# wenxiaoshuai/Points-Matching

Measured on AMD Instinct MI355X. Metric: descriptor-pair distances/s (BF-L2 2-NN + ratio stage); RANSAC hypotheses/s in `ransac`, higher is better.
Workload: dtype f32

## Files before the change

include/pm.h:

```cpp
#ifndef PM_H_
#define PM_H_

#include <stddef.h>
#include <stdint.h>

#ifdef __cplusplus
extern "C" {
#endif

#define PM_VERSION_MAJOR 0
#define PM_VERSION_MINOR 1

typedef enum pm_status {
    PM_OK            =  0,
    PM_E_INVALID     = -1,
    PM_E_TOO_FEW     = -2,
    PM_E_NO_MODEL    = -3,
    PM_E_HIP         = -4,
    PM_E_NOMEM       = -5,
    PM_E_UNSUPPORTED = -6
} pm_status;

typedef struct pm_match {
    int32_t queryIdx;
// ... 6 lines not shown

int  pm_ctx_create(int device, pm_ctx** out);
int  pm_ctx_destroy(pm_ctx* ctx);
int  pm_ctx_set_stream(pm_ctx* ctx, void* hip_stream);
int  pm_ctx_synchronize(pm_ctx* ctx);
int  pm_device_alloc(pm_ctx* ctx, size_t bytes, void** d_out);
int  pm_device_free(pm_ctx* ctx, void* d_ptr);
int  pm_device_upload(pm_ctx* ctx, void* d_dst, const void* src, size_t bytes);
int  pm_device_download(pm_ctx* ctx, void* dst, const void* d_src, size_t bytes);
int  pm_ctx_timing_enable(pm_ctx* ctx, int enable);
int  pm_ctx_timing_reset(pm_ctx* ctx);
int  pm_ctx_timing_get(pm_ctx* ctx, const char* kernel, double* mean_ms, int* launches);
int  pm_ctx_knn_diag_enable(pm_ctx* ctx, int enable);
int  pm_ctx_knn_stats(pm_ctx* ctx, int* rescans, int* nonfinite);
int  pm_ctx_knn_route(pm_ctx* ctx, int* route);
int  pm_ctx_filter_fusion_status(pm_ctx* ctx, int* gave_up);
enum {
    PM_OPT_RANSAC_PATH    = 1,
    PM_OPT_SCORE_OPERANDS = 2,
    PM_OPT_HAMMING_ROUTE  = 3,
    PM_OPT_KNN_F16_WAVES  = 4,
    PM_OPT_KNN_STAGING    = 6,
    PM_OPT_KNN_WG_PER_CU  = 7,
    PM_OPT_FILTER_FUSION  = 5,
    PM_OPT_KNN_XCD_TILE   = 8,
    PM_OPT_KNN_GENERAL_F16 = 9,
    PM_OPT_KNN_SEEDED     = 10,
    PM_OPT_KNN_U8_GROUP   = 11,
    PM_OPT_KNN_RING       = 12,
    PM_OPT_KNN_U8_REFINE  = 13,
    PM_OPT_KNN_RING_PROLOGUE = 14,
    PM_OPT_KNN_WIDE       = 15,
    PM_OPT_KNN_PREP_ROWS  = 16,
    PM_OPT_RANSAC_FORM    = 17,
    PM_OPT_RANSAC_WG_IDS  = 18,
    PM_OPT_HAMMING_REFINE = 19,
    PM_OPT_KNN_SUPERTILE  = 20,
    PM_OPT_FEAT_CAPACITY  = 21,
    PM_OPT_COUNT_         = 22
};
int  pm_ctx_set_option(pm_ctx* ctx, int option, int value);
int  pm_ctx_get_option(pm_ctx* ctx, int option, int* value);
const char* pm_last_error(void);
const char* pm_status_string(int status);
int  pm_version(void);

#define PM_MAX_K 16
#define PM_KNN_FORCE_EXACT  1
#define PM_KNN_FORCE_F32    2
#define PM_KNN_HINT_INTEGER 4
#define PM_KNN_HINT_U8      8
#define PM_KNN_HINT_UNIT_NORM 16
int pm_bf_knn_l2_f32(pm_ctx* ctx, const float* q, int nq, const float* t, int nt,
                     int dim, int k, int flags, pm_match* out);
// ... 379 lines not shown
```

points_matching_amd/api.py:

```python
import ctypes as C
import os

import numpy as np

_HERE = os.path.dirname(os.path.abspath(__file__))
LIB_PATH = os.environ.get("PM_LIB_PATH") or os.path.join(_HERE, "libpm_hip.so")

MATCH_DTYPE = np.dtype([("queryIdx", "<i4"), ("trainIdx", "<i4"), ("imgIdx", "<i4"),
                        ("distance", "<f4")])
PM_MAX_K = 16
PM_KNN_FORCE_EXACT = 1
PM_KNN_FORCE_F32 = 2
PM_KNN_HINT_INTEGER = 4
PM_KNN_HINT_U8 = 8
PM_KNN_HINT_UNIT_NORM = 16
PM_CROSS_RATIO_FWD = 1
PM_CROSS_RATIO_REV = 2
PM_GUIDE_F_SAMPSON = 0
PM_GUIDE_F_SYM = 1
PM_GUIDE_H = 2
PM_ERR_SAMPSON = 0
PM_ERR_SYM_EPIPOLAR = 1
PM_ERR_REPROJ = 2
PM_AFFINE_FULL = 0
PM_AFFINE_PARTIAL = 1
PM_OK, PM_E_INVALID, PM_E_TOO_FEW, PM_E_NO_MODEL, PM_E_HIP, PM_E_NOMEM, PM_E_UNSUPPORTED = \
    0, -1, -2, -3, -4, -5, -6

EXPORTS = [
    "pm_ctx_create", "pm_ctx_destroy", "pm_ctx_set_stream", "pm_ctx_synchronize",
    "pm_ctx_timing_enable", "pm_ctx_timing_reset", "pm_ctx_timing_get", "pm_ctx_knn_diag_enable", "pm_ctx_knn_stats", "pm_ctx_knn_route",
    "pm_ctx_filter_fusion_status",
    "pm_last_error",
    "pm_status_string", "pm_version",
    "pm_bf_knn_l2_f32", "pm_bf_knn_l2_f32_dev", "pm_bf_knn_hamming_u8", "pm_bf_knn_hamming_u8_dev",
    "pm_filter_midpoint", "pm_filter_ratio", "pm_match_indices", "pm_gather_points",
    "pm_format_match_list",
    "pm_filter_ratio_gather_dev", "pm_filter_midpoint_gather_dev", "pm_concat_points_dev",
    "pm_ransac_fundamental", "pm_ransac_score_dev", "pm_ransac_score_devn", "pm_ransac_model_from_hyp",
    "pm_ransac_model_from_key_dev", "pm_ransac_run_dev", "pm_ransac_shard_parts_dev", "pm_ransac_finish_parts_dev",
    "pm_ctx_set_option", "pm_ctx_get_option", "pm_bf_knn_l2_ratio_dev",
    "pm_flann_build", "pm_flann_destroy", "pm_flann_knn_l2_f32", "pm_flann_knn_l2_f32_dev", "pm_flann_export",
    "pm_mgpu_create", "pm_mgpu_destroy", "pm_mgpu_size", "pm_mgpu_ctx", "pm_mgpu_ransac_fundamental", "pm_mgpu_match_ransac",
    "pm_mgpu_lane_ctx", "pm_mgpu_set_lanes", "pm_mgpu_set_train", "pm_mgpu_set_train_dev", "pm_mgpu_submit_dev", "pm_mgpu_collect",
    "pm_mgpu_allgather_latency", "pm_mgpu_batch_run", "pm_mgpu_batch_set_option",
    "pm_batch_create", "pm_batch_destroy", "pm_batch_run", "pm_batch_set_option", "pm_batch_set_desc_type", "pm_batch_set_host_threads",
# ... 84 lines not shown
PM_OPT_KNN_STAGING = 6
PM_OPT_KNN_WG_PER_CU = 7
PM_OPT_KNN_XCD_TILE = 8
PM_OPT_KNN_GENERAL_F16 = 9
PM_OPT_KNN_SEEDED = 10
PM_OPT_KNN_U8_GROUP = 11
PM_OPT_KNN_RING = 12
PM_OPT_KNN_U8_REFINE = 13
PM_OPT_KNN_RING_PROLOGUE = 14
PM_OPT_KNN_WIDE = 15
PM_OPT_KNN_PREP_ROWS = 16
PM_OPT_RANSAC_FORM = 17
PM_OPT_RANSAC_WG_IDS = 18
PM_OPT_HAMMING_REFINE = 19
PM_OPT_KNN_SUPERTILE = 20
PM_OPT_FEAT_CAPACITY = 21


_lib = None


def lib():
    global _lib
    if _lib is None:
        if not os.path.exists(LIB_PATH):
            raise PmError(PM_E_UNSUPPORTED,
                          "%s is missing: run `python -m points_matching_amd.build`" % LIB_PATH)
        try:
            import torch
        except ImportError:
# ... 213 lines not shown
                                                mask_len, C.c_void_p(dninl_ptr or 0), C.c_void_p(dntotal_ptr or 0)))

    def knn_diag_enable(self, on=True):
        _check(lib().pm_ctx_knn_diag_enable(self._h, int(on)))

    def filter_fusion_gave_up(self):
        g = C.c_int()
        _check(lib().pm_ctx_filter_fusion_status(self._h, C.byref(g)))
        return g.value

    def knn_stats(self):
        r, nf = C.c_int(), C.c_int()
        _check(lib().pm_ctx_knn_stats(self._h, C.byref(r), C.byref(nf)))
        rt = C.c_int()
        _check(lib().pm_ctx_knn_route(self._h, C.byref(rt)))
        return {"rescans": r.value, "nonfinite": nf.value, "route": rt.value}

    def filter_ratio_gather_dev(self, dknn_ptr, nq, k, ratio, dkp1_ptr, dkp2_ptr, dgood_ptr, dxy1_ptr,
                                dxy2_ptr, dn_ptr):
        _check(lib().pm_filter_ratio_gather_dev(self._h, C.c_void_p(dknn_ptr), nq, k, C.c_float(ratio),
                                                C.c_void_p(dkp1_ptr), C.c_void_p(dkp2_ptr),
                                                C.c_void_p(dgood_ptr), C.c_void_p(dxy1_ptr),
                                                C.c_void_p(dxy2_ptr), C.c_void_p(dn_ptr)))

    def filter_cross_gather_dev(self, dfwd_ptr, nq, kf, drev_ptr, nt, kr, cross_flags, ratio, dkp1_ptr, dkp2_ptr, dgood_ptr,
                                dxy1_ptr, dxy2_ptr, dn_ptr):
        _check(lib().pm_filter_cross_gather_dev(self._h, C.c_void_p(dfwd_ptr), nq, kf, C.c_void_p(drev_ptr), nt, kr,
                                                cross_flags, C.c_float(ratio), C.c_void_p(dkp1_ptr or 0),
                                                C.c_void_p(dkp2_ptr or 0), C.c_void_p(dgood_ptr), C.c_void_p(dxy1_ptr or 0),
                                                C.c_void_p(dxy2_ptr or 0), C.c_void_p(dn_ptr)))

# ... 906 lines not shown
```

points_matching_amd/csrc/knn_l2.hip:

```cpp
#include <cstdlib>

#include "knn_shared.hpp"

namespace {

using namespace pm_knn;

constexpr int TILE_T = 64;
constexpr int PM_U8_FUSED_MAX_NQ = 768;
__host__ inline bool u8_fused_by_default(int nq) { return nq <= PM_U8_FUSED_MAX_NQ; }
constexpr float KNN_INF = __builtin_inff();

__device__ __forceinline__ uint32_t f32_bits(float f) { return __float_as_uint(f); }

__device__ __forceinline__ uint64_t knn_key(float dist, int idx)
{
    uint32_t b = (dist != dist) ? 0x7FC00000u : f32_bits(dist);
    return (static_cast<uint64_t>(b) << 32) | static_cast<uint32_t>(idx);
}

template <bool VEC4>
__device__ __forceinline__ float l2sqr_canonical(const float* __restrict__ a,
                                                 const float* __restrict__ b, int dim)
{
// ... 115 lines not shown
#pragma unroll
        for (int k = 0; k < 8; ++k) {
            float x = ALIGNED ? (k < 4 ? a[k & 3] : b[k & 3]) : e[k];
            const bool in = ALIGNED ? (c + (k & ~3) < dim) : (c + k < dim);
            v[k] = (live && in) ? x : 0.f;
        }
    }
};

template <bool SEEDED, int DP, bool ALIGNED>
__global__ __launch_bounds__(256) void knn_l2_prep16(const float* __restrict__ Q, int nq, int nq_pad,
                                                     const float* __restrict__ T, int nt, int nt_pad, int dim,
                                                     float* __restrict__ qnorm, float* __restrict__ tnorm,
                                                     _Float16* __restrict__ Qh, _Float16* __restrict__ Th,
                                                     float* __restrict__ seeds,
                                                     unsigned long long* __restrict__ stats, unsigned epoch)
{
    typedef F16Rows<DP> G;
    constexpr int ROWH = SEEDED ? DP : G::ROWH;
    constexpr int NCB = G::NCB;
    __shared__ unsigned wmax[4];
    __shared__ unsigned wbad[4];
    const int sub = threadIdx.x & 15, grp = threadIdx.x >> 4;
    const int qblocks = nq_pad / 64;
    const bool is_t = static_cast<int>(blockIdx.x) >= qblocks;
    const float* x = is_t ? T : Q;
    const int n = is_t ? nt : nq;
    float* norm = is_t ? tnorm : qnorm;
    _Float16* xh = is_t ? Th : Qh;
    const int row0 = (is_t ? blockIdx.x - qblocks : blockIdx.x) * 64;
    unsigned mx = 0u, bad = 0u;
// ... 59 lines not shown
        }
    }
#pragma unroll
    for (int o = 32; o > 0; o >>= 1) {
        mx = max(mx, static_cast<unsigned>(__shfl_xor(static_cast<int>(mx), o, 64)));
        bad |= static_cast<unsigned>(__shfl_xor(static_cast<int>(bad), o, 64));
    }
    if ((threadIdx.x & 63) == 0) { wmax[threadIdx.x >> 6] = mx; wbad[threadIdx.x >> 6] = bad; }
    __syncthreads();
    if (threadIdx.x == 0) {
        mx = max(max(wmax[0], wmax[1]), max(wmax[2], wmax[3]));
        bad = wbad[0] | wbad[1] | wbad[2] | wbad[3];
        const unsigned long long tag = static_cast<unsigned long long>(epoch) << 32;
        if (is_t) atomicMax(&stats[0], tag | mx);
        if (bad) atomicMax(&stats[1], tag | static_cast<unsigned long long>(bad == 1u ? 3u : bad));
    }
}

template <int ITERS>
__global__ __launch_bounds__(256) void knn_l2_prep8(const float* __restrict__ Q, int nq, int nq_pad,
                                                    const float* __restrict__ T, int nt, int nt_pad, int dim,
                                                    float* __restrict__ qnorm, float* __restrict__ tnorm,
                                                    uint2* __restrict__ Q8, uint2* __restrict__ T8,
                                                    int* __restrict__ seeds, unsigned long long* __restrict__ stats,
                                                    unsigned epoch, int t_wide, uint2* __restrict__ Qf)
{
    __shared__ unsigned wbad[4];
    const int sub = threadIdx.x & 15, grp = threadIdx.x >> 4;
    const int qblocks = nq_pad / (16 * ITERS);
    const bool is_t = static_cast<int>(blockIdx.x) >= qblocks;
// ... 318 lines not shown
        }
    }
#pragma unroll
    for (int o = 32; o > 0; o >>= 1) bad |= static_cast<unsigned>(__shfl_xor(static_cast<int>(bad), o, 64));
    if ((threadIdx.x & 63) == 0) wbad[threadIdx.x >> 6] = bad;
    __syncthreads();
    if (threadIdx.x == 0) {
        const unsigned long long tag = static_cast<unsigned long long>(epoch) << 32;
        bad = wbad[0] | wbad[1] | wbad[2] | wbad[3];
        if (blockIdx.x == 0) {
            atomicMax(&stats[0], tag | f32_bits(BOUND2));
            atomicMax(&stats[1], tag | 2ull);
        }
        if (bad) atomicMax(&stats[1], tag | 3ull);
    }
}

template <int KM>
struct BestN {
    uint64_t k[KM];
    float d[KM];
    __device__ __forceinline__ void init()
    {
#pragma unroll
        for (int i = 0; i < KM; ++i) { k[i] = ~0ull; d[i] = KNN_INF; }
    }
    __device__ __forceinline__ void insert(uint64_t key, float dist)
    {
        if (key < k[KM - 1]) {
            k[KM - 1] = key; d[KM - 1] = dist;
// ... 843 lines not shown
    }
    if (++ctx->kf_epoch >= (1u << 24)) {
        PM_HIP_CHECK(hipMemsetAsync(ctx->kf_tile, 0, static_cast<size_t>(ctx->kf_cap) * 12, ctx->stream));
        ctx->kf_epoch = 1;
    }
    fz.tile = ctx->kf_tile;
    fz.tilecnt = reinterpret_cast<unsigned*>(ctx->kf_tile + ctx->kf_cap);
    fz.err = reinterpret_cast<unsigned*>(ctx->knn_stats) + 12;
    fz.epoch = ctx->kf_epoch;
    return PM_OK;
}

int knn_l2_enqueue(pm_ctx* ctx, const float* dq, int nq, const float* dt, int nt, int dim, int k, int flags, pm_match* dout,
                   KnnFuse* fuse, const uint8_t* uq = nullptr, const uint8_t* ut = nullptr)
{
    const bool u8in = uq != nullptr;
    if (u8in) {
        const bool al = ((reinterpret_cast<uintptr_t>(uq) | reinterpret_cast<uintptr_t>(ut)) & 3) == 0;
        if (!(k <= 4 && (dim % 4) == 0 && dim <= 128 && nt >= 1 && al)) return 2;
        flags = PM_KNN_HINT_U8;
    }

    const bool aligned16 = u8in || ((reinterpret_cast<uintptr_t>(dq) | reinterpret_cast<uintptr_t>(dt)) & 15) == 0;
    const bool vec = (dim % 4) == 0 && aligned16;
    const bool narrow = vec && dim <= 128;
    const bool wide16 = !narrow && !(flags & PM_KNN_FORCE_F32) && ctx->opts[PM_OPT_KNN_WIDE] != 1;
    const bool fast = !(flags & PM_KNN_FORCE_EXACT) && (k <= 2 || (k <= 4 && ctx->opts[PM_OPT_KNN_WIDE] != 1)) && dim <= 256 &&
                      nt >= 1 && (narrow || wide16) && (dim >= 4 || !vec);
    if (!fast) {
        if (u8in) return 2;
// ... 114 lines not shown
    void* Qf = qfb ? pm::arena_take(ctx, qfb) : nullptr;
    PM_REQUIRE(qnorm && tnorm && (!want32 || cval32) && (!want16 || (cval16 && Qh && Th)) && (!sdb || seeds) && (!qfb || Qf),
               PM_E_NOMEM, "scratch arena too small");
    KnnFuse fz{};
    if (fuse) {
        fz = *fuse;
        fz.pk = static_cast<unsigned long long*>(pm::arena_take(ctx, pkb));
        PM_REQUIRE(fz.pk != nullptr, PM_E_NOMEM, "scratch arena too small");
        rc = kf_prepare(ctx, nq, fz, (u8r && u8_int_refine) ? 16 : 32);
        if (rc != PM_OK) return rc;
    }
    g32.cand = cval32;
    g16.cand = cval16;

    unsigned long long* stats = ctx->knn_stats;
    PM_REFUSE_CAPTURE(ctx);
    if (++ctx->knn_epoch == 0u) {
        PM_HIP_CHECK(hipMemsetAsync(stats, 0, 32, ctx->stream));
        ctx->knn_epoch = 1u;
    }
    const unsigned epoch = ctx->knn_epoch;
    unsigned* diag = nullptr;
    if (ctx->knn_diag) {
        diag = ctx->knn_diag_words;
        PM_HIP_CHECK(hipMemsetAsync(diag, 0, 12, ctx->stream));
    }
    {
        pm::ScopedKernelTime t(ctx, "knn_l2_prep");
        if (u8in)
            hipLaunchKernelGGL(knn_l2_prep8_u8, dim3(nq_pad / 64 + nt_pad / 64), dim3(256), 0, ctx->stream, uq, nq, nq_pad, ut, nt,
                               nt_pad, dim, qnorm, tnorm, reinterpret_cast<uint2*>(Qh), reinterpret_cast<uint2*>(Th),
                               static_cast<int*>(seeds), t_wide, static_cast<uint2*>(Qf));
        else if (u8r && ctx->opts[PM_OPT_KNN_PREP_ROWS] != 1)
            hipLaunchKernelGGL(knn_l2_prep8<1>, dim3(nq_pad / 16 + nt_pad / 16), dim3(256), 0, ctx->stream, dq, nq, nq_pad, dt,
                               nt, nt_pad, dim, qnorm, tnorm, reinterpret_cast<uint2*>(Qh), reinterpret_cast<uint2*>(Th),
                               static_cast<int*>(seeds), stats, epoch, t_wide, static_cast<uint2*>(Qf));
        else if (u8r)
            hipLaunchKernelGGL(knn_l2_prep8<4>, dim3(nq_pad / 64 + nt_pad / 64), dim3(256), 0, ctx->stream, dq, nq, nq_pad, dt,
                               nt, nt_pad, dim, qnorm, tnorm, reinterpret_cast<uint2*>(Qh), reinterpret_cast<uint2*>(Th),
                               static_cast<int*>(seeds), stats, epoch, t_wide, static_cast<uint2*>(Qf));
        else if (f16s)
            hipLaunchKernelGGL((knn_l2_prep16<true, 128, true>), dim3(nq_pad / 64 + nt_pad / 64), dim3(256), 0, ctx->stream, dq, nq,
                               nq_pad, dt, nt, nt_pad, dim, qnorm, tnorm, Qh, Th, static_cast<float*>(seeds), stats, epoch);
        else if (unit_hint) {
#define PM_PREP16U(DP_, AL_)                                                                                              \
    hipLaunchKernelGGL((knn_l2_prep16u<DP_, AL_>), dim3(nq_pad / 64 + nt_pad / 64), dim3(256), 0, ctx->stream, dq, nq, nq_pad, dt, \
                       nt, nt_pad, dim, qnorm, tnorm, Qh, Th, stats, epoch)
            if (dp16 == 128) { if (vec) PM_PREP16U(128, true); else PM_PREP16U(128, false); }
            else { if (vec) PM_PREP16U(256, true); else PM_PREP16U(256, false); }
#undef PM_PREP16U
        }
        else if (want16) {
#define PM_PREP16(DP_, AL_)                                                                                               \
    hipLaunchKernelGGL((knn_l2_prep16<false, DP_, AL_>), dim3(nq_pad / 64 + nt_pad / 64), dim3(256), 0, ctx->stream, dq, nq,    \
                       nq_pad, dt, nt, nt_pad, dim, qnorm, tnorm, Qh, Th, nullptr, stats, epoch)
            if (dp16 == 128) { if (vec) PM_PREP16(128, true); else PM_PREP16(128, false); }
            else { if (vec) PM_PREP16(256, true); else PM_PREP16(256, false); }
#undef PM_PREP16
        }
        else
            hipLaunchKernelGGL(knn_l2_prep, dim3((nq + 63) / 64 + (nt + 63) / 64), dim3(256), 0, ctx->stream, dq, nq, dt,
                               nt, dim, qnorm, tnorm, stats, epoch);
        if (route == ROUTE_AUTO && !gen32 && !unit_hint) {
#define PM_PREP16G(DP_, AL_)                                                                                              \
    hipLaunchKernelGGL((knn_l2_prep16g<DP_, AL_>), dim3(nq_pad / 64 + nt_pad / 64), dim3(256), 0, ctx->stream, dq, nq, nq_pad, dt, \
                       nt, nt_pad, dim, qnorm, tnorm, Qh, Th, stats, epoch)
            if (dp16 == 128) { if (vec) PM_PREP16G(128, true); else PM_PREP16G(128, false); }
            else { if (vec) PM_PREP16G(256, true); else PM_PREP16G(256, false); }
#undef PM_PREP16G
        }
        else if (gen32)
            hipLaunchKernelGGL(knn_gen_off, dim3(1), dim3(64), 0, ctx->stream, stats, epoch);
        PM_HIP_CHECK(hipGetLastError());
    }
    if (u8r) {
        rc = launch_coarse_u8(ctx, Qh, Qf, Th, static_cast<const int*>(seeds), nq, nq_pad, nt, splits16, g16.tiles_per_split,
                              reinterpret_cast<int*>(cval16), g16.slots, u8_group, u8_form);
        if (rc != PM_OK) return rc;
    } else if (f16s) {
        rc = launch_coarse_f16s(ctx, Qh, Th, static_cast<const float*>(seeds), nq, nq_pad, nt, splits16, g16.tiles_per_split,
                                ~g16.lid_mask, cval16, g16.slots);
        if (rc != PM_OK) return rc;
    } else if (want16) {
        rc = launch_coarse_f16(ctx, Qh, Th, nq, nq_pad, nt, splits16, g16.tiles_per_split, ~g16.lid_mask, cval16,
                               g16.slots, stats, epoch, route == ROUTE_AUTO ? 1 : 0, dp16);
        if (rc != PM_OK) return rc;
    }
    if (want32) {
        rc = launch_coarse_f32(ctx, dq, nq, dt, nt, dim, tnorm, splits32, g32.tiles_per_split, ~g32.lid_mask, cval32,
// ... 29 lines not shown
#define PM_REFINE4(VEC_, NS_, FUSE_, GEN_) do { if (k <= 2) PM_REFINE5(VEC_, NS_, FUSE_, GEN_, 2); else PM_REFINE5(VEC_, NS_, false, GEN_, 4); } while (0)
#define PM_REFINE3(NS_, FUSE_, GEN_) do { if (vec) PM_REFINE4(true, NS_, FUSE_, GEN_); else PM_REFINE4(false, NS_, FUSE_, GEN_); } while (0)
#define PM_REFINE2(NS_, FUSE_) do { if (route == ROUTE_AUTO) PM_REFINE3(NS_, FUSE_, true); else PM_REFINE3(NS_, FUSE_, false); } while (0)
#define PM_REFINE(NS_) do { if (fuse) PM_REFINE2(NS_, true); else PM_REFINE2(NS_, false); } while (0)
        if (max_slots <= 64) PM_REFINE(1);
        else if (max_slots <= 128) PM_REFINE(2);
        else if (max_slots <= 256) PM_REFINE(4);
        else PM_REFINE(8);
#undef PM_REFINE5
#undef PM_REFINE4
#undef PM_REFINE3
#undef PM_REFINE2
#undef PM_REFINE
        PM_HIP_CHECK(hipGetLastError());
    }
    return PM_OK;
}

}

extern "C" int pm_bf_knn_l2_f32_dev(pm_ctx* ctx, const float* dq, int nq, const float* dt, int nt, int dim,
                                    int k, int flags, pm_match* dout)
{
    PM_REQUIRE(ctx != nullptr, PM_E_INVALID, "ctx is null");
    PM_REQUIRE(nq >= 0 && nt >= 0 && dim >= 1 && k >= 1 && k <= PM_MAX_K, PM_E_INVALID,
               "need nq,nt >= 0, dim >= 1, 1 <= k <= PM_MAX_K");
    PM_REQUIRE(nq == 0 || (dq && dout), PM_E_INVALID, "null query/output pointer");
    PM_REQUIRE(nt == 0 || dt, PM_E_INVALID, "null train pointer");
    if (nq == 0) return PM_OK;
    PM_HIP_CHECK(hipSetDevice(ctx->device));
    return knn_l2_enqueue(ctx, dq, nq, dt, nt, dim, k, flags, dout, nullptr);
}

extern "C" int pm_bf_knn_l2_ratio_dev(pm_ctx* ctx, const float* d_q, int nq, const float* d_t, int nt, int dim, int flags,
                                      float ratio, const float* d_kp1_xy, const float* d_kp2_xy, pm_match* d_knn,
                                      pm_match* d_good, float* d_xy1, float* d_xy2, int32_t* d_n_good)
{
    PM_REQUIRE(ctx != nullptr && d_n_good != nullptr, PM_E_INVALID, "null argument");
    PM_REQUIRE(nq >= 0 && nt >= 0 && dim >= 1, PM_E_INVALID, "need nq,nt >= 0, dim >= 1");
    PM_REQUIRE(nq == 0 || (d_q && d_good), PM_E_INVALID, "null query/output pointer");
    PM_REQUIRE(nt == 0 || d_t, PM_E_INVALID, "null train pointer");
    PM_REQUIRE((d_kp1_xy == nullptr) == (d_kp2_xy == nullptr), PM_E_INVALID, "give both keypoint arrays or none");
    PM_REQUIRE(d_kp1_xy == nullptr || (d_xy1 && d_xy2), PM_E_INVALID, "null point outputs");
    PM_HIP_CHECK(hipSetDevice(ctx->device));
    if (nq == 0) {
        PM_HIP_CHECK(hipMemsetAsync(d_n_good, 0, sizeof(int32_t), ctx->stream));
        return PM_OK;
    }
    KnnFuse fz{};
    fz.ratio = ratio; fz.kp1 = d_kp1_xy; fz.kp2 = d_kp2_xy; fz.good = d_good; fz.xy1 = d_xy1; fz.xy2 = d_xy2; fz.n_out = d_n_good;
    const int fusion = ctx->opts[PM_OPT_FILTER_FUSION];
    const bool u8_hint = (flags & PM_KNN_HINT_U8) && !(flags & (PM_KNN_FORCE_F32 | PM_KNN_FORCE_EXACT));
    const bool separate = fusion == 1 || (fusion == 0 && d_knn != nullptr && !(u8_hint && u8_fused_by_default(nq)));
    int rc;
    if (!separate) {
        rc = knn_l2_enqueue(ctx, d_q, nq, d_t, nt, dim, 2, flags, d_knn, &fz);
        if (rc <= 0) return rc;
        return pm_filter_ratio_gather_dev(ctx, d_knn, nq, 2, ratio, d_kp1_xy, d_kp2_xy, d_good, d_xy1, d_xy2, d_n_good);
    }
// ... 24 lines not shown
    *ft = ctx->widen + a;
    return PM_OK;
}
}

extern "C" int pm_bf_knn_l2_u8_dev(pm_ctx* ctx, const uint8_t* dq, int nq, const uint8_t* dt, int nt, int dim, int k,
                                   pm_match* dout)
{
    PM_REQUIRE(ctx != nullptr, PM_E_INVALID, "ctx is null");
    PM_REQUIRE(nq >= 0 && nt >= 0 && dim >= 1 && k >= 1 && k <= PM_MAX_K, PM_E_INVALID,
               "need nq,nt >= 0, dim >= 1, 1 <= k <= PM_MAX_K");
    PM_REQUIRE(nq == 0 || (dq && dout), PM_E_INVALID, "null query/output pointer");
    PM_REQUIRE(nt == 0 || dt, PM_E_INVALID, "null train pointer");
    if (nq == 0) return PM_OK;
    PM_HIP_CHECK(hipSetDevice(ctx->device));
    int rc = nt >= 1 ? knn_l2_enqueue(ctx, nullptr, nq, nullptr, nt, dim, k, 0, dout, nullptr, dq, dt) : 2;
    if (rc != 2) return rc;
    const float *fq = nullptr, *ft = nullptr;
    rc = u8_widened(ctx, dq, nq, dt, nt, dim, &fq, &ft);
    if (rc != PM_OK) return rc;
    return knn_l2_enqueue(ctx, fq, nq, ft, nt, dim, k, PM_KNN_HINT_INTEGER, dout, nullptr);
}

extern "C" int pm_bf_knn_l2_u8_ratio_dev(pm_ctx* ctx, const uint8_t* d_q, int nq, const uint8_t* d_t, int nt, int dim, float ratio,
                                         const float* d_kp1_xy, const float* d_kp2_xy, pm_match* d_knn, pm_match* d_good,
                                         float* d_xy1, float* d_xy2, int32_t* d_n_good)
{
    PM_REQUIRE(ctx != nullptr && d_n_good != nullptr && d_knn != nullptr, PM_E_INVALID, "null argument (the u8 form needs the record buffer)");
    PM_REQUIRE(nq >= 0 && nt >= 0 && dim >= 1, PM_E_INVALID, "need nq,nt >= 0, dim >= 1");
    PM_REQUIRE(nq == 0 || (d_q && d_good), PM_E_INVALID, "null query/output pointer");
    PM_REQUIRE((d_kp1_xy == nullptr) == (d_kp2_xy == nullptr), PM_E_INVALID, "give both keypoint arrays or none");
    PM_REQUIRE(d_kp1_xy == nullptr || (d_xy1 && d_xy2), PM_E_INVALID, "null point outputs");
    PM_HIP_CHECK(hipSetDevice(ctx->device));
    if (nq == 0) {
        PM_HIP_CHECK(hipMemsetAsync(d_n_good, 0, sizeof(int32_t), ctx->stream));
        return PM_OK;
    }
    const int fusion = ctx->opts[PM_OPT_FILTER_FUSION];
    if (fusion == 2 || (fusion == 0 && u8_fused_by_default(nq))) {
        KnnFuse fz{};
        fz.ratio = ratio; fz.kp1 = d_kp1_xy; fz.kp2 = d_kp2_xy; fz.good = d_good; fz.xy1 = d_xy1; fz.xy2 = d_xy2; fz.n_out = d_n_good;
        const int rf = nt >= 1 ? knn_l2_enqueue(ctx, nullptr, nq, nullptr, nt, dim, 2, 0, d_knn, &fz, d_q, d_t) : 2;
        if (rf != 2) return rf;
    }
    const int rc = pm_bf_knn_l2_u8_dev(ctx, d_q, nq, d_t, nt, dim, 2, d_knn);
    if (rc != PM_OK) return rc;
    return pm_filter_ratio_gather_dev(ctx, d_knn, nq, 2, ratio, d_kp1_xy, d_kp2_xy, d_good, d_xy1, d_xy2, d_n_good);
}
// ... 80 lines not shown
```

points_matching_amd/csrc/pm_capi.cpp:

```cpp
#include <cfloat>
#include <cmath>

#include "pm_common.hpp"

namespace pm {

static thread_local char g_err[512] = "";

void set_error(const char* fmt, ...)
{
    va_list ap;
    va_start(ap, fmt);
    vsnprintf(g_err, sizeof g_err, fmt, ap);
    va_end(ap);
}

int arena_reserve(pm_ctx* ctx, size_t bytes)
{
    if (bytes <= ctx->arena_cap) return PM_OK;
    PM_HIP_CHECK(hipStreamSynchronize(ctx->stream));
    if (ctx->arena) PM_HIP_CHECK(hipFree(ctx->arena));
    ctx->arena = nullptr;
    ctx->arena_cap = 0;
    size_t cap = align_up(bytes + bytes / 4, size_t(1) << 20);
// ... 102 lines not shown
    PM_HIP_CHECK(hipGetDeviceCount(&n));
    PM_REQUIRE(device >= 0 && device < n && device < PM_MAX_DEVICES, PM_E_INVALID, "no such HIP device");
    PM_HIP_CHECK(hipSetDevice(device));
    pm_ctx* c = new (std::nothrow) pm_ctx();
    PM_REQUIRE(c != nullptr, PM_E_NOMEM, "host allocation failed");
    c->device = device;
    hipDeviceProp_t prop;
    if (hipGetDeviceProperties(&prop, device) == hipSuccess) c->n_cu = prop.multiProcessorCount;
    hipError_t e = hipStreamCreateWithFlags(&c->own_stream, hipStreamNonBlocking);
    if (e != hipSuccess) {
        set_error("hipStreamCreate failed: %s", hipGetErrorString(e));
        delete c;
        return PM_E_HIP;
    }
    c->stream = c->own_stream;
    e = hipMalloc(reinterpret_cast<void**>(&c->knn_stats), 64);
    if (e == hipSuccess) e = hipMemset(c->knn_stats, 0, 64);
    if (e != hipSuccess) {
        set_error("hipMalloc failed: %s", hipGetErrorString(e));
        (void)hipStreamDestroy(c->own_stream);
        delete c;
        return PM_E_NOMEM;
    }
    c->knn_diag_words = reinterpret_cast<unsigned*>(c->knn_stats + 4);
    *out = c;
    return PM_OK;
}

int pm_ctx_destroy(pm_ctx* ctx)
{
    if (!ctx) return PM_OK;
    (void)hipSetDevice(ctx->device);
// ... 6 lines not shown
    if (ctx->sync_words) (void)hipFree(ctx->sync_words);
    if (ctx->kf_tile) (void)hipFree(ctx->kf_tile);
    if (ctx->widen) (void)hipFree(ctx->widen);
    if (ctx->feat) (void)hipFree(ctx->feat);
    if (ctx->pinned) (void)hipHostFree(ctx->pinned);
    if (ctx->own_stream) (void)hipStreamDestroy(ctx->own_stream);
    delete ctx;
    return PM_OK;
}

int pm_ctx_set_stream(pm_ctx* ctx, void* hip_stream)
{
    PM_REQUIRE(ctx != nullptr, PM_E_INVALID, "ctx is null");
    PM_HIP_CHECK(hipStreamSynchronize(ctx->stream));
    ctx->stream = hip_stream ? static_cast<hipStream_t>(hip_stream) : ctx->own_stream;
    return PM_OK;
}

int pm_ctx_synchronize(pm_ctx* ctx)
{
    PM_REQUIRE(ctx != nullptr, PM_E_INVALID, "ctx is null");
    PM_HIP_CHECK(hipStreamSynchronize(ctx->stream));
    return PM_OK;
}

int pm_device_alloc(pm_ctx* ctx, size_t bytes, void** d_out)
{
    PM_REQUIRE(ctx != nullptr && d_out != nullptr, PM_E_INVALID, "null argument");
    *d_out = nullptr;
    PM_HIP_CHECK(hipSetDevice(ctx->device));
// ... 59 lines not shown
    double ms = 0.0;
    int n = 0;
    if (it != ctx->timers.end()) {
        n = it->second.launches;
        ms = n ? it->second.total_ms / n : 0.0;
    }
    if (mean_ms) *mean_ms = ms;
    if (launches) *launches = n;
    return PM_OK;
}

int pm_ctx_set_option(pm_ctx* ctx, int option, int value)
{
    PM_REQUIRE(ctx != nullptr, PM_E_INVALID, "ctx is null");
    PM_REQUIRE(option >= 1 && option < PM_OPT_COUNT_, PM_E_INVALID, "unknown option");
    const int vmax = option == PM_OPT_FEAT_CAPACITY ? (1 << 28) : option == PM_OPT_RANSAC_WG_IDS ? 128 : option == PM_OPT_KNN_RING_PROLOGUE ? 8 : option == PM_OPT_KNN_RING ? 6 : (option == PM_OPT_KNN_F16_WAVES || option == PM_OPT_KNN_U8_GROUP || option == PM_OPT_KNN_SUPERTILE) ? 3 : 2;
    PM_REQUIRE(value >= 0 && value <= vmax, PM_E_INVALID,
               "option value out of range (0 = automatic, 1, 2; KNN_F16_WAVES, KNN_U8_GROUP, KNN_SUPERTILE: .. 3; FEAT_CAPACITY: .. 2^28)");
    ctx->opts[option] = value;
    return PM_OK;
}

int pm_ctx_get_option(pm_ctx* ctx, int option, int* value)
{
    PM_REQUIRE(ctx != nullptr && value != nullptr, PM_E_INVALID, "null argument");
    PM_REQUIRE(option >= 1 && option < PM_OPT_COUNT_, PM_E_INVALID, "unknown option");
    *value = ctx->opts[option];
    return PM_OK;
}

int pm_ctx_knn_diag_enable(pm_ctx* ctx, int enable)
{
    PM_REQUIRE(ctx != nullptr, PM_E_INVALID, "ctx is null");
// ... 7 lines not shown
    unsigned w = 0;
    PM_HIP_CHECK(hipStreamSynchronize(ctx->stream));
    PM_HIP_CHECK(hipMemcpy(&w, reinterpret_cast<const char*>(ctx->knn_stats) + 48, sizeof w, hipMemcpyDeviceToHost));
    *gave_up = (ctx->kf_epoch != 0u && w == ctx->kf_epoch) ? 1 : 0;
    return PM_OK;
}

int pm_ctx_knn_stats(pm_ctx* ctx, int* rescans, int* nonfinite)
{
    PM_REQUIRE(ctx != nullptr, PM_E_INVALID, "ctx is null");
    unsigned h[2] = {0, 0};
    PM_HIP_CHECK(hipStreamSynchronize(ctx->stream));
    PM_HIP_CHECK(hipMemcpy(h, ctx->knn_diag_words, sizeof h, hipMemcpyDeviceToHost));
    if (rescans) *rescans = static_cast<int>(h[0]);
    if (nonfinite) *nonfinite = static_cast<int>(h[1]);
    return PM_OK;
}

int pm_ctx_knn_route(pm_ctx* ctx, int* route)
{
    PM_REQUIRE(ctx != nullptr && route != nullptr, PM_E_INVALID, "null argument");
    unsigned h = 0;
    PM_HIP_CHECK(hipStreamSynchronize(ctx->stream));
    PM_HIP_CHECK(hipMemcpy(&h, ctx->knn_diag_words + 2, sizeof h, hipMemcpyDeviceToHost));
    *route = static_cast<int>(h);
    return PM_OK;
}


int pm_filter_midpoint(const pm_match* m, int n, double* min_out, double* max_out,
// ... 195 lines not shown
```

points_matching_amd/csrc/pm_common.hpp:

```cpp
#pragma once
#include <hip/hip_runtime.h>

#include <cstdarg>
#include <cstdint>
#include <cstdio>
#include <cstring>
#include <map>
#include <string>
#include <vector>

#include "pm.h"

namespace pm {

void set_error(const char* fmt, ...);

#define PM_HIP_CHECK(expr)                                                              \
    do {                                                                                \
        hipError_t e_ = (expr);                                                         \
        if (e_ != hipSuccess) {                                                         \
            ::pm::set_error("%s failed: %s (%s:%d)", #expr, hipGetErrorString(e_),      \
                            __FILE__, __LINE__);                                        \
            return PM_E_HIP;                                                            \
        }                                                                               \
// ... 31 lines not shown
    hipStream_t own_stream = nullptr;
    hipStream_t stream = nullptr;
    char* arena = nullptr;
    size_t arena_cap = 0;
    size_t arena_off = 0;
    void* pinned = nullptr;
    size_t pinned_cap = 0;
    bool timing = false;
    std::map<std::string, pm::KernelTimer> timers;
    std::vector<hipEvent_t> event_pool;
    int n_cu = 256;
    unsigned long long* knn_stats = nullptr;
    unsigned* knn_diag_words = nullptr;
    unsigned knn_epoch = 0;
    bool knn_diag = false;
    unsigned* fg_counts = nullptr;
    unsigned fg_epoch = 0;
    unsigned long long* kf_tile = nullptr;
    int kf_cap = 0;
    unsigned kf_epoch = 0;
    int* sync_words = nullptr;
    int opts[PM_OPT_COUNT_] = {};
    float* widen = nullptr;
    size_t widen_cap = 0;
    char* feat = nullptr;
    size_t feat_cap = 0;
    size_t feat_counter_off = 0;
    int feat_noct = 0;
    int feat_w[16] = {}, feat_h[16] = {};
    size_t feat_off[16] = {};
// ... 62 lines not shown
```

Baseline: 2284 billion.

## Reuse previous call's f16 scale statistics to fuse kNN prep into one speculative pass

The prep stage now remembers the previous call's train max-norm and integer/general flags in a double-buffered device record. On warm calls it runs a single prep16w kernel that converts to f16 with the guessed scale, instead of running prep16 followed by prep16g. A fix-up kernel (prep16f) checks the guess against this call's statistics and redoes the conversion only on a mismatch or bound violation. This is meant to remove one full read/convert pass over the descriptors. In exchange it adds an extra launch, more host state tied to the stream, and capture refusal in more entry points.

```diff
diff --git a/include/pm.h b/include/pm.h
--- a/include/pm.h
+++ b/include/pm.h
@@ -44,6 +44,7 @@
 int  pm_ctx_knn_diag_enable(pm_ctx* ctx, int enable);
 int  pm_ctx_knn_stats(pm_ctx* ctx, int* rescans, int* nonfinite);
 int  pm_ctx_knn_route(pm_ctx* ctx, int* route);
+int  pm_ctx_knn_scale_stats(pm_ctx* ctx, int* form, int* violations);
 int  pm_ctx_filter_fusion_status(pm_ctx* ctx, int* gave_up);
 enum {
     PM_OPT_RANSAC_PATH    = 1,
@@ -67,7 +68,8 @@
     PM_OPT_HAMMING_REFINE = 19,
     PM_OPT_KNN_SUPERTILE  = 20,
     PM_OPT_FEAT_CAPACITY  = 21,
-    PM_OPT_COUNT_         = 22
+    PM_OPT_KNN_SCALE_MEMORY = 22,
+    PM_OPT_COUNT_         = 23
 };
 int  pm_ctx_set_option(pm_ctx* ctx, int option, int value);
 int  pm_ctx_get_option(pm_ctx* ctx, int option, int* value);
diff --git a/points_matching_amd/api.py b/points_matching_amd/api.py
--- a/points_matching_amd/api.py
+++ b/points_matching_amd/api.py
@@ -29,7 +29,7 @@
 
 EXPORTS = [
     "pm_ctx_create", "pm_ctx_destroy", "pm_ctx_set_stream", "pm_ctx_synchronize",
-    "pm_ctx_timing_enable", "pm_ctx_timing_reset", "pm_ctx_timing_get", "pm_ctx_knn_diag_enable", "pm_ctx_knn_stats", "pm_ctx_knn_route",
+    "pm_ctx_timing_enable", "pm_ctx_timing_reset", "pm_ctx_timing_get", "pm_ctx_knn_diag_enable", "pm_ctx_knn_stats", "pm_ctx_knn_route", "pm_ctx_knn_scale_stats",
     "pm_ctx_filter_fusion_status",
     "pm_last_error",
     "pm_status_string", "pm_version",
@@ -144,6 +144,7 @@
 PM_OPT_RANSAC_WG_IDS = 18
 PM_OPT_HAMMING_REFINE = 19
 PM_OPT_KNN_SUPERTILE = 20
+PM_OPT_KNN_SCALE_MEMORY = 22
 PM_OPT_FEAT_CAPACITY = 21
 
 
@@ -387,7 +388,10 @@
         _check(lib().pm_ctx_knn_stats(self._h, C.byref(r), C.byref(nf)))
         rt = C.c_int()
         _check(lib().pm_ctx_knn_route(self._h, C.byref(rt)))
-        return {"rescans": r.value, "nonfinite": nf.value, "route": rt.value}
+        fm, vi = C.c_int(), C.c_int()
+        _check(lib().pm_ctx_knn_scale_stats(self._h, C.byref(fm), C.byref(vi)))
+        return {"rescans": r.value, "nonfinite": nf.value, "route": rt.value, "form": "warm" if fm.value else "cold",
+                "violations": vi.value}
 
     def filter_ratio_gather_dev(self, dknn_ptr, nq, k, ratio, dkp1_ptr, dkp2_ptr, dgood_ptr, dxy1_ptr,
                                 dxy2_ptr, dn_ptr):
diff --git a/points_matching_amd/csrc/knn_l2.hip b/points_matching_amd/csrc/knn_l2.hip
--- a/points_matching_amd/csrc/knn_l2.hip
+++ b/points_matching_amd/csrc/knn_l2.hip
@@ -153,7 +153,8 @@
                                                      float* __restrict__ qnorm, float* __restrict__ tnorm,
                                                      _Float16* __restrict__ Qh, _Float16* __restrict__ Th,
                                                      float* __restrict__ seeds,
-                                                     unsigned long long* __restrict__ stats, unsigned epoch)
+                                                     unsigned long long* __restrict__ stats, unsigned epoch,
+                                                     unsigned long long* __restrict__ rec)
 {
     typedef F16Rows<DP> G;
     constexpr int ROWH = SEEDED ? DP : G::ROWH;
@@ -243,6 +244,10 @@
         const unsigned long long tag = static_cast<unsigned long long>(epoch) << 32;
         if (is_t) atomicMax(&stats[0], tag | mx);
         if (bad) atomicMax(&stats[1], tag | static_cast<unsigned long long>(bad == 1u ? 3u : bad));
+        if (rec) {
+            if (is_t) atomicMax(&rec[0], tag | mx);
+            if (bad) atomicMax(&rec[2], tag | static_cast<unsigned long long>(bad == 1u ? 3u : bad));
+        }
     }
 }
 
@@ -591,6 +596,190 @@
         }
         if (bad) atomicMax(&stats[1], tag | 3ull);
     }
+}
+
+template <int DP, bool ALIGNED>
+__device__ __forceinline__ void prep16w_load(Row8<ALIGNED> (&ld)[4][F16Rows<DP>::NCB], const float* __restrict__ x, int n, int dim,
+                                             int row0)
+{
+    const int sub = threadIdx.x & 15, grp = threadIdx.x >> 4;
+#pragma unroll
+    for (int it = 0; it < 4; ++it) {
+        const int row = row0 + it * 16 + grp;
+        const float* p = x + static_cast<size_t>(row < n ? row : n - 1) * dim;
+#pragma unroll
+        for (int cb = 0; cb < F16Rows<DP>::NCB; ++cb) ld[it][cb].load(p, 128 * cb + 8 * sub, dim);
+    }
+}
+
+template <int DP, bool ALIGNED, bool general>
+__device__ __forceinline__ void prep16w_group(const Row8<ALIGNED> (&ld)[4][F16Rows<DP>::NCB], int ht, int n, int dim,
+                                              float* __restrict__ norm, _Float16* __restrict__ xh, bool is_t, int row0,
+                                              unsigned& mx, unsigned& bad, unsigned& viol)
+{
+    typedef F16Rows<DP> G;
+    constexpr int NCB = G::NCB;
+    const int sub = threadIdx.x & 15, grp = threadIdx.x >> 4;
+    const int c0 = 8 * sub;
+    const float st = __builtin_ldexpf(1.f, 10 - ht);
+    const float bound2 = __builtin_ldexpf(1.f, 2 * ht);
+#pragma unroll
+    for (int it = 0; it < 4; ++it) {
+        const int row = row0 + it * 16 + grp;
+        const bool live = row < n;
+        float s = 0.f;
+        bool okrow = true;
+#pragma unroll
+        for (int cb = 0; cb < NCB; ++cb) {
+            float v[8];
+            ld[it][cb].get(128 * cb + c0, dim, live, v);
+#pragma unroll
+            for (int e = 0; e < 8; ++e) {
+                s = fmaf(v[e], v[e], s);
+                okrow &= (v[e] == __builtin_rintf(v[e])) && (__builtin_fabsf(v[e]) <= G::MAXABS);
+            }
+        }
+#pragma unroll
+        for (int o = 8; o > 0; o >>= 1) s += __shfl_xor(s, o, 16);
+        if (!okrow) bad |= 2u;
+        QueryScale qs{};
+        if constexpr (general) qs = query_scale(ht, s);
+        const float sc = !general ? 1.f : (is_t ? st : qs.sq);
+        const bool zero = !live || (general && !is_t && qs.unranked);
+#pragma unroll
+        for (int cb = 0; cb < NCB; ++cb) {
+            float v[8];
+            ld[it][cb].get(128 * cb + c0, dim, !zero, v);
+            f16x8 hv;
+#pragma unroll
+            for (int e = 0; e < 8; ++e) hv[e] = static_cast<_Float16>(v[e] * sc);
+            *reinterpret_cast<f16x8*>(xh + static_cast<size_t>(row) * G::ROWH + 128 * cb + c0) = hv;
+        }
+        if (sub == 0) {
+            if (live) {
+                norm[row] = s;
+                if (!(s < KNN_INF)) bad |= 3u;
+                else if (is_t) {
+                    mx = max(mx, f32_bits(s));
+                    if (general && !(s < bound2)) ++viol;
+                }
+            }
+            f16x8 e0 = {0, 0, 0, 0, 0, 0, 0, 0};
+            const f16x8 e1 = {0, 0, 0, 0, 0, 0, 0, 0};
+            if (is_t) {
+                if (live) {
+                    const float z = general ? __builtin_rintf(s * st * st * 16.f) : s;
+                    const unsigned tn = z < 16777216.f ? static_cast<unsigned>(z) : (general ? 16777215u : 0u);
+                    e0[0] = static_cast<_Float16>(static_cast<float>(tn >> 13));
+                    e0[1] = static_cast<_Float16>(static_cast<float>((tn >> 6) & 127u));
+                    e0[2] = static_cast<_Float16>(static_cast<float>(tn & 63u));
+                } else {
+                    e0[0] = static_cast<_Float16>(60000.f);
+                    if (general) e0[1] = static_cast<_Float16>(60000.f);
+                }
+            } else if (general && live && qs.unranked) {
+                e0[0] = static_cast<_Float16>(__builtin_nanf(""));
+            } else {
+                e0[0] = static_cast<_Float16>(general ? qs.qc[0] : -4096.f);
+                e0[1] = static_cast<_Float16>(general ? qs.qc[1] : -32.f);
+                e0[2] = static_cast<_Float16>(general ? qs.qc[2] : -0.5f);
+            }
+            *reinterpret_cast<f16x8*>(xh + static_cast<size_t>(row) * G::ROWH + DP) = e0;
+            *reinterpret_cast<f16x8*>(xh + static_cast<size_t>(row) * G::ROWH + DP + 8) = e1;
+        }
+    }
+}
+
+struct ScaleGuess {
+    bool general;
+    int ht;
+};
+__device__ __forceinline__ ScaleGuess scale_guess(const unsigned long long* __restrict__ rec, int rslot, unsigned prev_epoch)
+{
+    const unsigned long long r0 = rec[rslot], r2 = rec[2 + rslot];
+    const float pmax = static_cast<unsigned>(r0 >> 32) == prev_epoch ? __uint_as_float(static_cast<unsigned>(r0)) : 0.f;
+    ScaleGuess g;
+    g.general = static_cast<unsigned>(r2 >> 32) == prev_epoch && (r2 & 2ull) && pmax > 0.f;
+    g.ht = g.general ? half_exp_ceil(pmax * 1.001954078674316f) : 10;
+    return g;
+}
+
+template <int DP, bool ALIGNED>
+__global__ __launch_bounds__(256) void knn_l2_prep16w(const float* __restrict__ Q, int nq, int nq_pad,
+                                                      const float* __restrict__ T, int nt, int nt_pad, int dim,
+                                                      float* __restrict__ qnorm, float* __restrict__ tnorm,
+                                                      _Float16* __restrict__ Qh, _Float16* __restrict__ Th,
+                                                      unsigned long long* __restrict__ stats, unsigned epoch,
+                                                      unsigned long long* __restrict__ rec, int rslot, unsigned prev_epoch,
+                                                      unsigned* __restrict__ diag)
+{
+    __shared__ unsigned wmax[4], wbad[4], wviol[4];
+    const int qblocks = nq_pad / 64;
+    const bool is_t = static_cast<int>(blockIdx.x) >= qblocks;
+    const int row0 = (is_t ? blockIdx.x - qblocks : blockIdx.x) * 64;
+    Row8<ALIGNED> ld[4][F16Rows<DP>::NCB];
+    prep16w_load<DP, ALIGNED>(ld, is_t ? T : Q, is_t ? nt : nq, dim, row0);
+    const ScaleGuess g = scale_guess(rec, rslot, prev_epoch);
+    unsigned long long* recw = rec + (rslot ^ 1);
+    unsigned mx = 0u, bad = 0u, viol = 0u;
+    if (g.general)
+        prep16w_group<DP, ALIGNED, true>(ld, g.ht, is_t ? nt : nq, dim, is_t ? tnorm : qnorm, is_t ? Th : Qh, is_t, row0, mx, bad, viol);
+    else
+        prep16w_group<DP, ALIGNED, false>(ld, g.ht, is_t ? nt : nq, dim, is_t ? tnorm : qnorm, is_t ? Th : Qh, is_t, row0, mx, bad, viol);
+#pragma unroll
+    for (int o = 32; o > 0; o >>= 1) {
+        mx = max(mx, static_cast<unsigned>(__shfl_xor(static_cast<int>(mx), o, 64)));
+        bad |= static_cast<unsigned>(__shfl_xor(static_cast<int>(bad), o, 64));
+        viol += static_cast<unsigned>(__shfl_xor(static_cast<int>(viol), o, 64));
+    }
+    if ((threadIdx.x & 63) == 0) { wmax[threadIdx.x >> 6] = mx; wbad[threadIdx.x >> 6] = bad; wviol[threadIdx.x >> 6] = viol; }
+    __syncthreads();
+    if (threadIdx.x == 0) {
+        const unsigned long long tag = static_cast<unsigned long long>(epoch) << 32;
+        mx = max(max(wmax[0], wmax[1]), max(wmax[2], wmax[3]));
+        bad = wbad[0] | wbad[1] | wbad[2] | wbad[3];
+        viol = wviol[0] + wviol[1] + wviol[2] + wviol[3];
+        if (is_t) {
+            atomicMax(&recw[0], tag | mx);
+            atomicMax(&stats[0], tag | (g.general ? max(mx, f32_bits(__builtin_ldexpf(1.f, 2 * g.ht - 2))) : mx));
+        }
+        if (bad) {
+            const unsigned long long f = tag | static_cast<unsigned long long>(bad == 1u ? 3u : bad);
+            atomicMax(&stats[1], f);
+            atomicMax(&recw[2], f);
+        }
+        if (viol) {
+            atomicMax(&recw[4], tag | 1ull);
+            if (diag) atomicAdd(&diag[3], viol);
+        }
+    }
+}
+
+template <int DP, bool ALIGNED>
+__global__ __launch_bounds__(256) void knn_l2_prep16f(const float* __restrict__ Q, int nq, int nq_pad,
+                                                      const float* __restrict__ T, int nt, int nt_pad, int dim,
+                                                      float* __restrict__ qnorm, float* __restrict__ tnorm,
+                                                      _Float16* __restrict__ Qh, _Float16* __restrict__ Th, unsigned epoch,
+                                                      const unsigned long long* __restrict__ rec, int rslot, unsigned prev_epoch)
+{
+    const ScaleGuess g = scale_guess(rec, rslot, prev_epoch);
+    const unsigned long long* recw = rec + (rslot ^ 1);
+    const unsigned long long m0 = recw[0], m2 = recw[2], m4 = recw[4];
+    const unsigned flags = static_cast<unsigned>(m2 >> 32) == epoch ? static_cast<unsigned>(m2) : 0u;
+    const bool data_general = (flags & 2u) != 0u, violated = static_cast<unsigned>(m4 >> 32) == epoch;
+    if ((flags & 1u) || (data_general == g.general && !violated)) return;
+    const float tmax = static_cast<unsigned>(m0 >> 32) == epoch ? __uint_as_float(static_cast<unsigned>(m0)) : 0.f;
+    const int ht = tmax > 0.f ? half_exp_ceil(tmax) : 10;
+    const int qblocks = nq_pad / 64;
+    const bool is_t = static_cast<int>(blockIdx.x) >= qblocks;
+    const int row0 = (is_t ? blockIdx.x - qblocks : blockIdx.x) * 64;
+    unsigned d0 = 0u, d1 = 0u, d2 = 0u;
+    Row8<ALIGNED> ld[4][F16Rows<DP>::NCB];
+    prep16w_load<DP, ALIGNED>(ld, is_t ? T : Q, is_t ? nt : nq, dim, row0);
+    if (data_general)
+        prep16w_group<DP, ALIGNED, true>(ld, ht, is_t ? nt : nq, dim, is_t ? tnorm : qnorm, is_t ? Th : Qh, is_t, row0, d0, d1, d2);
+    else
+        prep16w_group<DP, ALIGNED, false>(ld, ht, is_t ? nt : nq, dim, is_t ? tnorm : qnorm, is_t ? Th : Qh, is_t, row0, d0, d1, d2);
 }
 
 template <int KM>
@@ -1464,6 +1653,10 @@
 int knn_l2_enqueue(pm_ctx* ctx, const float* dq, int nq, const float* dt, int nt, int dim, int k, int flags, pm_match* dout,
                    KnnFuse* fuse, const uint8_t* uq = nullptr, const uint8_t* ut = nullptr)
 {
+    PM_REFUSE_CAPTURE(ctx);
+    const bool sm_prev = ctx->sm_valid && ctx->sm_stream == ctx->stream;
+    ctx->sm_valid = false;
+    if (ctx->knn_diag) ctx->knn_last_form = 0;
     const bool u8in = uq != nullptr;
     if (u8in) {
         const bool al = ((reinterpret_cast<uintptr_t>(uq) | reinterpret_cast<uintptr_t>(ut)) & 3) == 0;
@@ -1608,17 +1801,23 @@
     g16.cand = cval16;
 
     unsigned long long* stats = ctx->knn_stats;
-    PM_REFUSE_CAPTURE(ctx);
+    unsigned long long* rec = stats + 8;
+    bool warm = sm_prev;
     if (++ctx->knn_epoch == 0u) {
         PM_HIP_CHECK(hipMemsetAsync(stats, 0, 32, ctx->stream));
+        PM_HIP_CHECK(hipMemsetAsync(rec, 0, 48, ctx->stream));
         ctx->knn_epoch = 1u;
+        warm = false;
     }
     const unsigned epoch = ctx->knn_epoch;
     unsigned* diag = nullptr;
     if (ctx->knn_diag) {
         diag = ctx->knn_diag_words;
-        PM_HIP_CHECK(hipMemsetAsync(diag, 0, 12, ctx->stream));
-    }
+        PM_HIP_CHECK(hipMemsetAsync(diag, 0, 16, ctx->stream));
+    }
+    const bool sm_call = route == ROUTE_AUTO && !unit_hint && !gen32;
+    warm = warm && sm_call && ctx->opts[PM_OPT_KNN_SCALE_MEMORY] != 1;
+    const int sm_wslot = ctx->sm_slot ^ 1;
     {
         pm::ScopedKernelTime t(ctx, "knn_l2_prep");
         if (u8in)
@@ -1635,7 +1834,7 @@
                                static_cast<int*>(seeds), stats, epoch, t_wide, static_cast<uint2*>(Qf));
         else if (f16s)
             hipLaunchKernelGGL((knn_l2_prep16<true, 128, true>), dim3(nq_pad / 64 + nt_pad / 64), dim3(256), 0, ctx->stream, dq, nq,
-                               nq_pad, dt, nt, nt_pad, dim, qnorm, tnorm, Qh, Th, static_cast<float*>(seeds), stats, epoch);
+                               nq_pad, dt, nt, nt_pad, dim, qnorm, tnorm, Qh, Th, static_cast<float*>(seeds), stats, epoch, nullptr);
         else if (unit_hint) {
 #define PM_PREP16U(DP_, AL_)                                                                                              \
     hipLaunchKernelGGL((knn_l2_prep16u<DP_, AL_>), dim3(nq_pad / 64 + nt_pad / 64), dim3(256), 0, ctx->stream, dq, nq, nq_pad, dt, \
@@ -1644,10 +1843,20 @@
             else { if (vec) PM_PREP16U(256, true); else PM_PREP16U(256, false); }
 #undef PM_PREP16U
         }
+        else if (warm) {
+#define PM_PREP16W(DP_, AL_)                                                                                              \
+    hipLaunchKernelGGL((knn_l2_prep16w<DP_, AL_>), dim3(nq_pad / 64 + nt_pad / 64), dim3(256), 0, ctx->stream, dq, nq, nq_pad, dt, \
+                       nt, nt_pad, dim, qnorm, tnorm, Qh, Th, stats, epoch, rec, ctx->sm_slot, ctx->sm_epoch, diag);                 \
+    hipLaunchKernelGGL((knn_l2_prep16f<DP_, AL_>), dim3(nq_pad / 64 + nt_pad / 64), dim3(256), 0, ctx->stream, dq, nq, nq_pad, dt, \
+                       nt, nt_pad, dim, qnorm, tnorm, Qh, Th, epoch, rec, ctx->sm_slot, ctx->sm_epoch)
+            if (dp16 == 128) { if (vec) { PM_PREP16W(128, true); } else { PM_PREP16W(128, false); } }
+            else { if (vec) { PM_PREP16W(256, true); } else { PM_PREP16W(256, false); } }
+#undef PM_PREP16W
+        }
         else if (want16) {
 #define PM_PREP16(DP_, AL_)                                                                                               \
     hipLaunchKernelGGL((knn_l2_prep16<false, DP_, AL_>), dim3(nq_pad / 64 + nt_pad / 64), dim3(256), 0, ctx->stream, dq, nq,    \
-                       nq_pad, dt, nt, nt_pad, dim, qnorm, tnorm, Qh, Th, nullptr, stats, epoch)
+                       nq_pad, dt, nt, nt_pad, dim, qnorm, tnorm, Qh, Th, nullptr, stats, epoch, sm_call ? rec + sm_wslot : nullptr)
             if (dp16 == 128) { if (vec) PM_PREP16(128, true); else PM_PREP16(128, false); }
             else { if (vec) PM_PREP16(256, true); else PM_PREP16(256, false); }
 #undef PM_PREP16
@@ -1655,7 +1864,7 @@
         else
             hipLaunchKernelGGL(knn_l2_prep, dim3((nq + 63) / 64 + (nt + 63) / 64), dim3(256), 0, ctx->stream, dq, nq, dt,
                                nt, dim, qnorm, tnorm, stats, epoch);
-        if (route == ROUTE_AUTO && !gen32 && !unit_hint) {
+        if (route == ROUTE_AUTO && !gen32 && !unit_hint && !warm) {
 #define PM_PREP16G(DP_, AL_)                                                                                              \
     hipLaunchKernelGGL((knn_l2_prep16g<DP_, AL_>), dim3(nq_pad / 64 + nt_pad / 64), dim3(256), 0, ctx->stream, dq, nq, nq_pad, dt, \
                        nt, nt_pad, dim, qnorm, tnorm, Qh, Th, stats, epoch)
@@ -1667,6 +1876,7 @@
             hipLaunchKernelGGL(knn_gen_off, dim3(1), dim3(64), 0, ctx->stream, stats, epoch);
         PM_HIP_CHECK(hipGetLastError());
     }
+    if (ctx->knn_diag) ctx->knn_last_form = warm ? 1 : 0;
     if (u8r) {
         rc = launch_coarse_u8(ctx, Qh, Qf, Th, static_cast<const int*>(seeds), nq, nq_pad, nt, splits16, g16.tiles_per_split,
                               reinterpret_cast<int*>(cval16), g16.slots, u8_group, u8_form);
@@ -1726,6 +1936,12 @@
 #undef PM_REFINE
         PM_HIP_CHECK(hipGetLastError());
     }
+    if (sm_call) {
+        ctx->sm_slot = sm_wslot;
+        ctx->sm_epoch = epoch;
+        ctx->sm_stream = ctx->stream;
+        ctx->sm_valid = true;
+    }
     return PM_OK;
 }
 
@@ -1755,6 +1971,7 @@
     PM_REQUIRE((d_kp1_xy == nullptr) == (d_kp2_xy == nullptr), PM_E_INVALID, "give both keypoint arrays or none");
     PM_REQUIRE(d_kp1_xy == nullptr || (d_xy1 && d_xy2), PM_E_INVALID, "null point outputs");
     PM_HIP_CHECK(hipSetDevice(ctx->device));
+    PM_REFUSE_CAPTURE(ctx);
     if (nq == 0) {
         PM_HIP_CHECK(hipMemsetAsync(d_n_good, 0, sizeof(int32_t), ctx->stream));
         return PM_OK;
@@ -1809,6 +2026,7 @@
     PM_REQUIRE(nt == 0 || dt, PM_E_INVALID, "null train pointer");
     if (nq == 0) return PM_OK;
     PM_HIP_CHECK(hipSetDevice(ctx->device));
+    PM_REFUSE_CAPTURE(ctx);
     int rc = nt >= 1 ? knn_l2_enqueue(ctx, nullptr, nq, nullptr, nt, dim, k, 0, dout, nullptr, dq, dt) : 2;
     if (rc != 2) return rc;
     const float *fq = nullptr, *ft = nullptr;
@@ -1827,6 +2045,7 @@
     PM_REQUIRE((d_kp1_xy == nullptr) == (d_kp2_xy == nullptr), PM_E_INVALID, "give both keypoint arrays or none");
     PM_REQUIRE(d_kp1_xy == nullptr || (d_xy1 && d_xy2), PM_E_INVALID, "null point outputs");
     PM_HIP_CHECK(hipSetDevice(ctx->device));
+    PM_REFUSE_CAPTURE(ctx);
     if (nq == 0) {
         PM_HIP_CHECK(hipMemsetAsync(d_n_good, 0, sizeof(int32_t), ctx->stream));
         return PM_OK;
diff --git a/points_matching_amd/csrc/pm_capi.cpp b/points_matching_amd/csrc/pm_capi.cpp
--- a/points_matching_amd/csrc/pm_capi.cpp
+++ b/points_matching_amd/csrc/pm_capi.cpp
@@ -140,8 +140,8 @@
         return PM_E_HIP;
     }
     c->stream = c->own_stream;
-    e = hipMalloc(reinterpret_cast<void**>(&c->knn_stats), 64);
-    if (e == hipSuccess) e = hipMemset(c->knn_stats, 0, 64);
+    e = hipMalloc(reinterpret_cast<void**>(&c->knn_stats), 128);
+    if (e == hipSuccess) e = hipMemset(c->knn_stats, 0, 128);
     if (e != hipSuccess) {
         set_error("hipMalloc failed: %s", hipGetErrorString(e));
         (void)hipStreamDestroy(c->own_stream);
@@ -178,6 +178,7 @@
     PM_REQUIRE(ctx != nullptr, PM_E_INVALID, "ctx is null");
     PM_HIP_CHECK(hipStreamSynchronize(ctx->stream));
     ctx->stream = hip_stream ? static_cast<hipStream_t>(hip_stream) : ctx->own_stream;
+    ctx->sm_valid = false;
     return PM_OK;
 }
 
@@ -267,9 +268,9 @@
 {
     PM_REQUIRE(ctx != nullptr, PM_E_INVALID, "ctx is null");
     PM_REQUIRE(option >= 1 && option < PM_OPT_COUNT_, PM_E_INVALID, "unknown option");
-    const int vmax = option == PM_OPT_FEAT_CAPACITY ? (1 << 28) : option == PM_OPT_RANSAC_WG_IDS ? 128 : option == PM_OPT_KNN_RING_PROLOGUE ? 8 : option == PM_OPT_KNN_RING ? 6 : (option == PM_OPT_KNN_F16_WAVES || option == PM_OPT_KNN_U8_GROUP || option == PM_OPT_KNN_SUPERTILE) ? 3 : 2;
+    const int vmax = option == PM_OPT_FEAT_CAPACITY ? (1 << 28) : option == PM_OPT_KNN_SCALE_MEMORY ? 1 : option == PM_OPT_RANSAC_WG_IDS ? 128 : option == PM_OPT_KNN_RING_PROLOGUE ? 8 : option == PM_OPT_KNN_RING ? 6 : (option == PM_OPT_KNN_F16_WAVES || option == PM_OPT_KNN_U8_GROUP || option == PM_OPT_KNN_SUPERTILE) ? 3 : 2;
     PM_REQUIRE(value >= 0 && value <= vmax, PM_E_INVALID,
-               "option value out of range (0 = automatic, 1, 2; KNN_F16_WAVES, KNN_U8_GROUP, KNN_SUPERTILE: .. 3; FEAT_CAPACITY: .. 2^28)");
+               "option value out of range (0 = automatic, 1, 2; KNN_SCALE_MEMORY: .. 1; KNN_F16_WAVES, KNN_U8_GROUP, KNN_SUPERTILE: .. 3; FEAT_CAPACITY: .. 2^28)");
     ctx->opts[option] = value;
     return PM_OK;
 }
@@ -307,6 +308,17 @@
     PM_HIP_CHECK(hipMemcpy(h, ctx->knn_diag_words, sizeof h, hipMemcpyDeviceToHost));
     if (rescans) *rescans = static_cast<int>(h[0]);
     if (nonfinite) *nonfinite = static_cast<int>(h[1]);
+    return PM_OK;
+}
+
+int pm_ctx_knn_scale_stats(pm_ctx* ctx, int* form, int* violations)
+{
+    PM_REQUIRE(ctx != nullptr, PM_E_INVALID, "ctx is null");
+    unsigned h = 0;
+    PM_HIP_CHECK(hipStreamSynchronize(ctx->stream));
+    PM_HIP_CHECK(hipMemcpy(&h, ctx->knn_diag_words + 3, sizeof h, hipMemcpyDeviceToHost));
+    if (form) *form = ctx->knn_last_form;
+    if (violations) *violations = static_cast<int>(h);
     return PM_OK;
 }
 
diff --git a/points_matching_amd/csrc/pm_common.hpp b/points_matching_amd/csrc/pm_common.hpp
--- a/points_matching_amd/csrc/pm_common.hpp
+++ b/points_matching_amd/csrc/pm_common.hpp
@@ -69,6 +69,11 @@
     unsigned* knn_diag_words = nullptr;
     unsigned knn_epoch = 0;
     bool knn_diag = false;
+    bool sm_valid = false;
+    int sm_slot = 0;
+    unsigned sm_epoch = 0;
+    hipStream_t sm_stream = nullptr;
+    int knn_last_form = 0;
     unsigned* fg_counts = nullptr;
     unsigned fg_epoch = 0;
     unsigned long long* kf_tile = nullptr;
```

New measurement: 2325 billion (median of 3 runs). 1.02x the previous value.
